# open-mmlab/Live2Diff

Measured on AMD Instinct MI355X. Metric: frames/sec @512×512, 2 denoise steps; per-step latency; 1/2/4/8 GPU, higher is better.
Workload: dtype f16; 1 GPU; BASELINE configs[1]: 512x512 image (64x64 latent), 2 denoise steps, KV window L=16 (8 sink + 8 rolling), SD-1.5 UNet widths + Live2Diff temporal attention, one independent stream per GPU; plan_launches=433, hipgraph=False, device=AMD Radeon Graphics (gfx950:sramecc+:xnack-, 256 CUs), output_finite=True, default_workload=True

## Files before the change

### live2diff_amd/csrc/igemm.hip

```cpp
#include "common.h"

typedef unsigned int u32x4 __attribute__((ext_vector_type(4)));
#define L2D_GPTR(p) ((__attribute__((address_space(1))) const void *)(p))
#define L2D_LPTR(p) ((__attribute__((address_space(3))) void *)(p))

struct IGemmArgs {
    const h16 *w;
    const h16 *zero;
    long long sw;
    int Nout, Kp, nwg, ntn, ntm, order, splitk;
    float inv_ntn, inv_ntm, inv_s;
    const h16 *x1, *x2;
    long long sx1;
    int M, C1, C2, ldx1, ldx2, CinP, B, Hin, Win, Hout, Wout, stride, ups, taps;
    int pad;
    float inv_hw, inv_wout;
    const float *bias, *rowbias;
    const h16 *res;
    h16 *out;
    long long so, sres;
    int ldo, ldr, ldrb, rows_per_bias, epi, epl;
    float *ws;
    unsigned int *cnt;
    unsigned long long *gn1, *gn2;
    int gnT, gnG, cpg1, choff1, cpg2, choff2;
#ifdef L2D_PROBES
    unsigned long long *probe;
#endif
};

#ifdef L2D_PROBES
static unsigned long long *g_igemm_probe = nullptr;
extern "C" void l2d_igemm_set_probe(void *p) { g_igemm_probe = (unsigned long long *)p; }
#define L2D_STAMP(i)                                                                                              \
    do {                                                                                                          \
        if (a.probe && threadIdx.x == 0)                                                                          \
            a.probe[((blockIdx.z * gridDim.y + blockIdx.y) * (unsigned long long)gridDim.x + blockIdx.x) * 8 + (i)] = __builtin_readcyclecounter(); \
    } while (0)
#else
#define L2D_STAMP(i) do { } while (0)
#endif

__device__ __forceinline__ int l2d_divf(int n, int d, float inv) {
    int q = (int)((float)n * inv);
    const int r = n - q * d;
    q += (r >= d ? 1 : 0) - (r < 0 ? 1 : 0);
    return q;
}

__device__ __forceinline__ void igemm_epilogue(const IGemmArgs &a, h16 *outp, const h16 *resp, int m, int n, f32x4 v) {
    const float *rb = a.rowbias ? a.rowbias + (long long)(m / a.rows_per_bias) * a.ldrb : nullptr;
    if (n + 4 > a.Nout) {
#pragma unroll
        for (int r = 0; r < 4; ++r) {
            if (n + r >= a.Nout) break;
            float y = v[r];
            if (a.bias) y += a.bias[n + r];
            if (rb) y += rb[n + r];
            if (a.epi == 2) y = l2d_silu(y);
            if (a.epi == 3) y = fmaxf(y, 0.f);
            if (a.epi == 5) y = l2d_gelu(y);
            if (resp) y += (float)resp[(long long)m * a.ldr + n + r];
            if (a.epi == 4) y = fmaxf(y, 0.f);
            outp[(long long)m * a.ldo + n + r] = (h16)y;
        }
        return;
    }
    if (a.bias) v += *reinterpret_cast<const f32x4 *>(a.bias + n);
    if (rb) v += *reinterpret_cast<const f32x4 *>(rb + n);
    if (a.epi == 2) {
#pragma unroll
        for (int r = 0; r < 4; ++r) v[r] = l2d_silu(v[r]);
    }
    if (a.epi == 3) {
#pragma unroll
        for (int r = 0; r < 4; ++r) v[r] = fmaxf(v[r], 0.f);
    }
    if (a.epi == 5) {
#pragma unroll
        for (int r = 0; r < 4; ++r) v[r] = l2d_gelu(v[r]);
    }
    if (resp) {
        h16x4 rr = *reinterpret_cast<const h16x4 *>(resp + (long long)m * a.ldr + n);
#pragma unroll
        for (int r = 0; r < 4; ++r) v[r] += (float)rr[r];
    }
    if (a.epi == 4) {
#pragma unroll
        for (int r = 0; r < 4; ++r) v[r] = fmaxf(v[r], 0.f);
    }
    h16x4 o;
#pragma unroll
    for (int r = 0; r < 4; ++r) o[r] = (h16)v[r];
    *reinterpret_cast<h16x4 *>(outp + (long long)m * a.ldo + n) = o;
}

template <int TN, int TM, int MODE, int BK, int NS>
__global__ __launch_bounds__(256, (TN == 128 && BK == 32) ? (NS == 2 ? 4 : 3) : 1) void igemm_kernel(IGemmArgs a) {
    constexpr int NI = TN / 32;
    constexpr int MI = TM / 32;
    constexpr int SPR = BK / 8;
    constexpr int RPI = 64 / SPR;
    constexpr int NIW = TN / RPI / 4;
    constexpr int NIX = TM / RPI / 4;
    constexpr int LPS = NIW + NIX;
    constexpr int KK = BK / 32;
    constexpr int STAGE = (TN + TM) * BK;
    extern __shared__ __attribute__((aligned(16))) h16 smem[];

    unsigned ka0, ka1, ka2, ka3;
    {
        const auto kp = __builtin_amdgcn_kernarg_segment_ptr();
        static_assert(sizeof(IGemmArgs) > 0xc0 + 4, "argument block shrank: adjust the warm-up offsets");
        asm volatile("s_load_dword %0, %4, 0x0\n\ts_load_dword %1, %4, 0x40\n\ts_load_dword %2, %4, 0x80\n\ts_load_dword %3, %4, 0xc0"
                     : "=&s"(ka0), "=&s"(ka1), "=&s"(ka2), "=&s"(ka3)
                     : "s"(kp));
    }
    L2D_STAMP(0);
    const int tid = threadIdx.x;
    const int lane = tid & 63;
    const int wave = __builtin_amdgcn_readfirstlane(tid >> 6);
    const int wn = wave >> 1, wm = wave & 1;
    const int li = lane & 15, lg = lane >> 4;
    auto swz = [](int r) { return BK == 32 ? ((r >> 1) & 3) : (BK == 64 ? (r & 7) : (r & 15)); };

// ... 180 lines not shown
        if (resp) {
#pragma unroll
            for (int it = 0; it < EPI_IT; ++it) {
                const int c = it * 256 + tid, row = c / CPRN, cc = c % CPRN;
                const int m = m0 + row, n = n0 + cc * 8;
                resv[RES_EARLY ? it : 0] = (m < a.M && n < a.Nout) ? l2d_ld8(resp + (long long)m * a.ldr + n) : l2d_zero8();
            }
        }
    };
    if (vec && RES_EARLY && !split) load_early();
    if (kb < ke) issue_x();

    f32x4 acc[NI][MI];
#pragma unroll
    for (int i = 0; i < NI; ++i)
#pragma unroll
        for (int j = 0; j < MI; ++j) acc[i][j] = (f32x4){0.f, 0.f, 0.f, 0.f};

    int aoff[KK][NI], boff[KK][MI];
#pragma unroll
    for (int kk = 0; kk < KK; ++kk) {
#pragma unroll
        for (int i = 0; i < NI; ++i) {
            const int r = wn * (TN / 2) + i * 16 + li;
            aoff[kk][i] = r * BK + (((kk * 4 + lg) ^ swz(r)) << 3);
        }
#pragma unroll
        for (int j = 0; j < MI; ++j) {
            const int r = wm * (TM / 2) + j * 16 + li;
            boff[kk][j] = (TN + r) * BK + (((kk * 4 + lg) ^ swz(r)) << 3);
        }
    }
    int cp_slot = 0;
    auto compute = [&]() {
        const h16 *st = smem + cp_slot * STAGE;
#pragma unroll
        for (int kk = 0; kk < KK; ++kk) {
            h16x8 af[NI], bf[MI];
#pragma unroll
            for (int i = 0; i < NI; ++i) af[i] = l2d_ld8(st + aoff[kk][i]);
#pragma unroll
            for (int j = 0; j < MI; ++j) bf[j] = l2d_ld8(st + boff[kk][j]);
#pragma unroll
            for (int i = 0; i < NI; ++i)
#pragma unroll
                for (int j = 0; j < MI; ++j)
                    acc[i][j] = __builtin_amdgcn_mfma_f32_16x16x32_f16(af[i], bf[j], acc[i][j], 0, 0, 0);
        }
        cp_slot = (cp_slot + 1 == NS) ? 0 : cp_slot + 1;
    };

#pragma unroll
    for (int s = 1; s < NS - 1; ++s)
        if (kb + s < ke) issue();
    L2D_STAMP(2);
    int kt = kb;
    for (; kt + (NS - 1) < ke; ++kt) {
        asm volatile("s_waitcnt vmcnt(%0)" ::"n"((NS - 2) * LPS) : "memory");
        __builtin_amdgcn_s_barrier();
        if (kt == kb) L2D_STAMP(3);
        issue();
        compute();
    }
    for (; kt < ke; ++kt) {
        asm volatile("s_waitcnt vmcnt(0)" ::: "memory");
        __builtin_amdgcn_s_barrier();
        compute();
    }

    L2D_STAMP(4);
    if (split && a.cnt) {
        const int S = a.splitk;
        constexpr int AUX_SC1 = 16;
        float *slab = a.ws + ((z * nwg + wgid) * S) * (long long)(TN * TM);
        const __amdgpu_buffer_rsrc_t rs = __builtin_amdgcn_make_buffer_rsrc(slab, 0, S * TN * TM * 4, 0x00020000);
        const int mine = ((int)blockIdx.y * (TN * TM) + tid * 4) * 4;
#pragma unroll
        for (int j = 0; j < MI; ++j) {
            if (m0 + wm * (TM / 2) + j * 16 >= a.M) continue;
#pragma unroll
            for (int i = 0; i < NI; ++i)
                __builtin_amdgcn_raw_buffer_store_b128(__builtin_bit_cast(u32x4, acc[i][j]), rs, mine + (i * MI + j) * 4096, 0, AUX_SC1);
        }
        asm volatile("s_waitcnt vmcnt(0)" ::: "memory");
        __syncthreads();
        unsigned int *flag = reinterpret_cast<unsigned int *>(smem);
        if (tid == 0) *flag = atomicAdd(a.cnt + (z * nwg + wgid), 1u);
        __syncthreads();
        const bool last = (*flag == (unsigned int)(S - 1));
        __syncthreads();
        if (!last) return;
        if (tid == 0) atomicExch(a.cnt + (z * nwg + wgid), 0u);
#pragma unroll
        for (int i = 0; i < NI; ++i)
#pragma unroll
            for (int j = 0; j < MI; ++j) acc[i][j] = (f32x4){0.f, 0.f, 0.f, 0.f};
#pragma unroll
        for (int j = 0; j < MI; ++j) {
            if (m0 + wm * (TM / 2) + j * 16 >= a.M) continue;
#pragma unroll 4
            for (int y = 0; y < S; ++y) {
                const int src = (y * (TN * TM) + tid * 4) * 4;
#pragma unroll
                for (int i = 0; i < NI; ++i)
                    acc[i][j] += __builtin_bit_cast(f32x4, __builtin_amdgcn_raw_buffer_load_b128(rs, src + (i * MI + j) * 4096, 0, AUX_SC1));
            }
        }
        if (vec && RES_EARLY) load_early();
    } else if (split) {
        const int NoutP = (a.Nout + 3) & ~3;
        float *wsp = a.ws + ((long long)z * a.splitk + blockIdx.y) * a.M * NoutP;
#pragma unroll
        for (int j = 0; j < MI; ++j) {
            const int m = m0 + wm * (TM / 2) + j * 16 + li;
            if (m >= a.M) continue;
#pragma unroll
            for (int i = 0; i < NI; ++i) {
                const int n = n0 + wn * (TN / 2) + i * 16 + lg * 4;
                if (n >= a.Nout) continue;
                *reinterpret_cast<f32x4 *>(wsp + (long long)m * NoutP + n) = acc[i][j];
            }
        }
        return;
    }
    if (vec) {
        const int pitch = (a.epi == 1 ? TN / 2 : TN) + 8;
        h16 *ot = smem;
        if (!RES_EARLY) load_bias();
        __syncthreads();
        if (a.epi == 1) {
#pragma unroll
            for (int j = 0; j < MI; ++j) {
                const int row = wm * (TM / 2) + j * 16 + li;
#pragma unroll
                for (int p = 0; p < NI / 2; ++p) {
                    const int col = wn * (TN / 4) + p * 16 + lg * 4;
                    h16x4 o;
#pragma unroll
                    for (int r = 0; r < 4; ++r) {
                        const float v = acc[2 * p][j][r] + biasv[2 * p][r];
                        const float g = acc[2 * p + 1][j][r] + biasv[2 * p + 1][r];
                        o[r] = (h16)(v * l2d_gelu(g));
                    }
                    *reinterpret_cast<h16x4 *>(ot + row * pitch + col) = o;
                }
            }
        } else {
#pragma unroll
            for (int j = 0; j < MI; ++j) {
                const int row = wm * (TM / 2) + j * 16 + li;
                const float *rb = (a.rowbias && !rb_in_bias)
                                      ? a.rowbias + (long long)((m0 + row < a.M ? m0 + row : a.M - 1) / a.rows_per_bias) * a.ldrb
                                      : nullptr;
#pragma unroll
                for (int i = 0; i < NI; ++i) {
                    const int col = wn * (TN / 2) + i * 16 + lg * 4;
                    f32x4 v = acc[i][j] + biasv[i];
                    if constexpr (RES_EARLY) v += rbv[i];
                    if (rb && n0 + col < a.Nout) v += *reinterpret_cast<const f32x4 *>(rb + n0 + col);
                    if (a.epi == 2) {
#pragma unroll
                        for (int r = 0; r < 4; ++r) v[r] = l2d_silu(v[r]);
                    }
                    if (a.epi == 3) {
#pragma unroll
                        for (int r = 0; r < 4; ++r) v[r] = fmaxf(v[r], 0.f);
                    }
                    if (a.epi == 5) {
#pragma unroll
                        for (int r = 0; r < 4; ++r) v[r] = l2d_gelu(v[r]);
                    }
                    h16x4 o;
#pragma unroll
                    for (int r = 0; r < 4; ++r) o[r] = (h16)v[r];
                    *reinterpret_cast<h16x4 *>(ot + row * pitch + col) = o;
                }
            }
        }
        constexpr int CPRN_LOG = (CPRN == 16) ? 4 : 3;
        const int cshift = (a.epi == 1) ? CPRN_LOG - 1 : CPRN_LOG;
        const int n0o = (a.epi == 1) ? (n0 >> 1) : n0;
        L2D_STAMP(5);
        h16x8 rlate[RES_EARLY ? 1 : EPI_IT];
        if (!RES_EARLY && resp) {
#pragma unroll
            for (int it = 0; it < EPI_IT; ++it) {
                const int c = it * 256 + tid, row = c / CPRN, cc = c % CPRN;
                const int m = m0 + row, n = n0 + cc * 8;
                rlate[it] = (m < a.M && n < a.Nout) ? l2d_ld8(resp + (long long)m * a.ldr + n) : l2d_zero8();
            }
        }
// ... 255 lines not shown
```

### live2diff_amd/csrc/rowgemm.hip

```cpp
#include <type_traits>

#include "common.h"

typedef float f32x16 __attribute__((ext_vector_type(16)));

struct RowGemmArgs {
    const h16 *x, *w;
    const float *bias;
    const h16 *res;
    h16 *out, *outT;
    const long long *gnacc;
    unsigned long long *gn1, *gn2;
    long long sT;
    int M, K, Nout, ldx, ldo, ldr, ldt;
    int epi, pro, T, G, cpg;
    int nm, ny, ytr, tr_n0, order;
    int gnT, gnG, cpg1, choff1, cpg2, choff2;
    float eps, inv_cpg;
#ifdef L2D_PROBES
    unsigned long long *probe;
#endif
};

#ifdef L2D_PROBES
// ... 188 lines not shown
    for (int e = 0; e < 4; ++e) { gs[e] = 0.f; gq[e] = 0.f; }
    const h16x2 ones2 = {(h16)1.0f, (h16)1.0f};
#pragma unroll
    for (int it = 0; it < EIT; ++it) {
        const int row = rr + it * RPP;
        if (!on || row >= BM || m0 + row >= a.M) continue;
        h16x8 v = l2d_ld8(os + row * pitch + cc * 8);
        if (a.res) {
            if constexpr (RES_PRE) v = v + resv[it];
            else v = v + l2d_ld8(a.res + (long long)(m0 + row) * a.ldr + nb_o + cc * 8);
        }
        l2d_st8_out<L2D_WT_ROWGEMM>(a.out + (long long)(m0 + row) * a.ldo + nb_o + cc * 8, v);
        if (gn) {
#pragma unroll
            for (int e = 0; e < 4; ++e) {
                const h16x2 pr = {v[2 * e], v[2 * e + 1]};
                gs[e] = __builtin_amdgcn_fdot2(pr, ones2, gs[e], false);
                gq[e] = __builtin_amdgcn_fdot2(pr, pr, gq[e], false);
            }
        }
    }
    RG_STAMP(6);
    if (gn) {
        float *red = reinterpret_cast<float *>(smem + BM * pitch);
#pragma unroll
        for (int e = 0; e < 4; ++e) { red[tid * 8 + e] = gs[e]; red[tid * 8 + 4 + e] = gq[e]; }
        __syncthreads();
        float *chs1 = red + nthr * 8, *chs2 = chs1 + (BNo >> 1);
        if (tid < (BNo >> 1)) {
            const int c8 = tid >> 2, e = tid & 3;
            float s = 0.f, q = 0.f;
            for (int r = 0; r < RPP; ++r) { s += red[(r * CPR + c8) * 8 + e]; q += red[(r * CPR + c8) * 8 + 4 + e]; }
            chs1[tid] = s; chs2[tid] = q;
        }
        __syncthreads();
        const int bsmp = m0 / a.gnT;
        l2d_gn_flush(a.gn1, a.gnG, a.cpg1 >> 1, a.choff1 >> 1, bsmp, chs1, chs2, nb_o >> 1, BNo >> 1, tid);
        l2d_gn_flush(a.gn2, a.gnG, a.cpg2 >> 1, a.choff2 >> 1, bsmp, chs1, chs2, nb_o >> 1, BNo >> 1, tid);
    }
}

template <int NT, int MT, int RD, int SK, int MAXT>
__global__ __launch_bounds__(MAXT) void rowgemm_kernel(RowGemmArgs a) {
    constexpr int BM = 32 * MT;
    extern __shared__ __attribute__((aligned(16))) h16 smem[];
    const int tid = threadIdx.x, lane = tid & 63;
    const int nthr = blockDim.x, NW = nthr >> 6;
    const int wave = __builtin_amdgcn_readfirstlane(tid >> 6);
    RG_STAMP(0);

    const int nwg = a.nm * a.ny;
    int wgid;
    {
        const int q = nwg >> 3, r = nwg & 7, xcd = blockIdx.x & 7, idx = blockIdx.x >> 3;
        wgid = (xcd < r ? xcd * (q + 1) : r * (q + 1) + (xcd - r) * q) + idx;
    }
    int mtile, y;
    if (a.order) { y = wgid / a.nm; mtile = wgid - y * a.nm; }
    else { mtile = wgid / a.ny; y = wgid - mtile * a.ny; }
    const int m0 = mtile * BM;
    const int S = SK > 0 ? SK : (a.K >> 4);
    const int KK = SK > 0 ? SK * 16 : a.K;
    const int t0 = (y * NW + wave) * NT;

    const h16 *wp = a.w + (long long)t0 * S * 512;
    const int wlane = lane * 8;
    const long long tstride = (long long)S * 512;
    constexpr int RING = rg_ring<RD, SK>();
    h16x8 wr[RING][NT];
    auto request_ring = [&]() {
        long long ro = 0;
#pragma unroll
        for (int s = 0; s < RING; ++s) {
            asm volatile("" : "+s"(ro));
#pragma unroll
            for (int i = 0; i < NT; ++i) wr[s][i] = l2d_ld8(wp + (ro + i * tstride) + wlane);
            ro += 512;
        }
        __builtin_amdgcn_sched_barrier(0);
    };
    RG_STAMP(1);

    float *tab = reinterpret_cast<float *>(smem + BM * KK + 8 * BM);
    if (a.pro == 2) {
        float *rstd_s = tab + 2 * KK, *shf_s = rstd_s + 32;
        if (tid < a.G) {
            const long long *src = a.gnacc + ((long long)(m0 / a.T) * a.G + tid) * 2;
            const float s = (float)((double)src[0] * (1.0 / 1048576.0));
            const float q = (float)((double)src[1] * (1.0 / 4096.0));
            const float inv = 1.0f / ((float)a.T * (float)a.cpg);
            const float mean = s * inv;
            const float var = fmaxf(q * inv - mean * mean, 0.f);
            const float rstd = rsqrtf(var + a.eps);
            rstd_s[tid] = rstd;
            shf_s[tid] = -mean * rstd;
        }
        __syncthreads();
        for (int c = tid; c < KK; c += nthr) {
            const int g = (int)(((float)c + 0.5f) * a.inv_cpg);
            tab[c] = rstd_s[g];
            tab[KK + c] = shf_s[g];
        }
        __syncthreads();
    }

    RG_STAMP(2);
    {
        constexpr int XG = 10;
        const bool wide = nthr >= 16 * BM && (KK & 127) == 0;
        const int lsh = wide ? 4 : 3, LPR = 1 << lsh;
        const int KS = KK >> (3 + lsh);
        const int nch = (KS + XG - 1) / XG;
        const int j = tid & (LPR - 1);
        const int dstep = 8 * LPR * BM;
        const int r0 = tid >> lsh, rstep = nthr >> lsh;
        const bool has_row = r0 < BM;
        const int r_last = has_row ? r0 + ((BM - 1 - r0) / rstep) * rstep : 0;
        const bool ln_reg = a.pro == 1 && nch == 1;

        auto load_group = [&](h16x8 (&v)[XG], int r, int i0) {
            const int m = m0 + r;
            const h16 *src = a.x + (long long)(m < a.M ? m : 0) * a.ldx + j * 8;
#pragma unroll
            for (int u = 0; u < XG; ++u) v[u] = l2d_ld8(src + (i0 + u < KS ? i0 + u : KS - 1) * (8 * LPR));
            __builtin_amdgcn_sched_barrier(0);
        };
        auto consume_group = [&](h16x8 (&v)[XG], int r, int i0, float &s) {
            const bool rv = m0 + r < a.M;
            h16 *dst = smem + (j * BM + (r ^ (2 * (j & 7)))) * 8;
            if (ln_reg) {
                float t = 0.f;
#pragma unroll
                for (int u = 0; u < XG; ++u) {
                    if (u >= KS) break;
                    if (!rv) v[u] = l2d_zero8();
#pragma unroll
                    for (int e = 0; e < 8; ++e) t += (float)v[u][e];
                }
                const float mean = rg_row_sum(t, wide) / (float)KK;
                float q = 0.f;
#pragma unroll
                for (int u = 0; u < XG; ++u) {
                    if (u >= KS) break;
#pragma unroll
                    for (int e = 0; e < 8; ++e) { const float d = (float)v[u][e] - mean; q += d * d; }
                }
                const float rstd = rsqrtf(rg_row_sum(q, wide) / (float)KK + a.eps);
#pragma unroll
                for (int u = 0; u < XG; ++u) {
                    if (u >= KS) break;
                    h16x8 o;
#pragma unroll
                    for (int e = 0; e < 8; ++e) o[e] = (h16)(((float)v[u][e] - mean) * rstd);
                    l2d_st8(dst + u * dstep, o);
                }
                return;
            }
#pragma unroll
            for (int u = 0; u < XG; ++u) {
                if (i0 + u >= KS) break;
                if (!rv) v[u] = l2d_zero8();
                if (a.pro == 2) {
                    const int c0 = (j + LPR * (i0 + u)) * 8;
                    const f32x4 sa = *reinterpret_cast<const f32x4 *>(tab + c0), sb = *reinterpret_cast<const f32x4 *>(tab + c0 + 4);
                    const f32x4 ha = *reinterpret_cast<const f32x4 *>(tab + KK + c0), hb = *reinterpret_cast<const f32x4 *>(tab + KK + c0 + 4);
                    h16x8 o;
#pragma unroll
                    for (int e = 0; e < 4; ++e) {
                        o[e] = (h16)((float)v[u][e] * sa[e] + ha[e]);
                        o[4 + e] = (h16)((float)v[u][4 + e] * sb[e] + hb[e]);
                    }
                    v[u] = rv ? o : l2d_zero8();
                } else if (a.pro == 1) {
#pragma unroll
                    for (int e = 0; e < 8; ++e) s += (float)v[u][e];
                }
                l2d_st8(dst + (i0 + u) * dstep, v[u]);
            }
        };
        auto finish_row_lds = [&](int r, float s) {
            h16 *dst = smem + (j * BM + (r ^ (2 * (j & 7)))) * 8;
            const float mean = rg_row_sum(s, wide) / (float)KK;
            float q = 0.f;
#pragma unroll 5
            for (int i = 0; i < KS; ++i) {
                const h16x8 v = l2d_ld8(dst + i * dstep);
#pragma unroll
                for (int e = 0; e < 8; ++e) { const float d = (float)v[e] - mean; q += d * d; }
            }
            const float rstd = rsqrtf(rg_row_sum(q, wide) / (float)KK + a.eps);
#pragma unroll 5
            for (int i = 0; i < KS; ++i) {
                const h16x8 v = l2d_ld8(dst + i * dstep);
                h16x8 o;
#pragma unroll
                for (int e = 0; e < 8; ++e) o[e] = (h16)(((float)v[e] - mean) * rstd);
                l2d_st8(dst + i * dstep, o);
            }
        };

        float srow = 0.f;
        if (has_row) {
            for (int r = r0; r < BM; r += rstep) {
                const int ng = (r == r_last) ? nch - 1 : nch;
                for (int c = 0; c < ng; ++c) {
                    h16x8 v[XG];
                    load_group(v, r, c * XG);
                    consume_group(v, r, c * XG, srow);
                }
                if (r != r_last) {
                    if (a.pro == 1 && !ln_reg) finish_row_lds(r, srow);
                    srow = 0.f;
                }
            }
        }
        h16x8 vl[XG];
        if (has_row) load_group(vl, r_last, (nch - 1) * XG);
        request_ring();
        if (has_row) {
            consume_group(vl, r_last, (nch - 1) * XG, srow);
            if (a.pro == 1 && !ln_reg) finish_row_lds(r_last, srow);
        }
    }
    __syncthreads();
    RG_STAMP(3);
    rowgemm_body<NT, MT, RD, SK>(a, smem, wr, wp, wlane, tstride, S, m0, y, NW, wave, lane, tid, nthr);
}

template <int NT, int MT, int RD, int SK, int MAXT>
static void launch_rg(const RowGemmArgs &a, int nthr, size_t lds, hipStream_t s) {
    static bool attr_done_dev[L2D_MAX_DEV] = {false};
    bool &attr_done = attr_done_dev[l2d_dev_ordinal()];
    if (lds > 65536 && !attr_done) {
        if (hipFuncSetAttribute((const void *)rowgemm_kernel<NT, MT, RD, SK, MAXT>, hipFuncAttributeMaxDynamicSharedMemorySize, 163840) == hipSuccess)
            attr_done = true;
        else
            (void)hipGetLastError();
    }
    hipLaunchKernelGGL((rowgemm_kernel<NT, MT, RD, SK, MAXT>), dim3(a.nm * a.ny), dim3(nthr), lds, s, a);
}

template <int NT, int MT, int RD, int MAXT>
static void launch_k(const RowGemmArgs &a, int nthr, size_t lds, hipStream_t s) {
    switch (a.K) {
        case 320: launch_rg<NT, MT, RD, 20, MAXT>(a, nthr, lds, s); break;
        case 640: launch_rg<NT, MT, RD, 40, MAXT>(a, nthr, lds, s); break;
        case 1280: launch_rg<NT, MT, RD, 80, MAXT>(a, nthr, lds, s); break;
        default: launch_rg<NT, MT, RD, 0, MAXT>(a, nthr, lds, s); break;
    }
}

int l2d_launch_rowgemm(const l2d_op *op, hipStream_t s) {
    RowGemmArgs a;
    a.x = (const h16 *)op->p[0]; a.w = (const h16 *)op->p[1]; a.bias = (const float *)op->p[2]; a.res = (const h16 *)op->p[3];
    a.out = (h16 *)op->p[4]; a.gnacc = (const long long *)op->p[7];
    a.outT = (h16 *)op->p[8];
    a.gn1 = (unsigned long long *)op->p[9]; a.gn2 = (unsigned long long *)op->p[10];
    a.M = op->i[0]; a.K = op->i[1]; a.Nout = op->i[2]; a.ldx = op->i[3]; a.ldo = op->i[4]; a.ldr = op->i[5];
    a.epi = op->i[6]; a.pro = op->i[7]; a.T = op->i[9]; a.G = op->i[10];
    const int NW = op->i[12], NT = op->i[13], MT = op->i[14];
    const int ntr = op->i[15];
    a.ldt = op->i[16]; a.order = op->i[17] ? 1 : 0;
    a.sT = op->l[0];
    a.eps = op->f[0];
#ifdef L2D_PROBES
    a.probe = g_rowgemm_probe;
#endif
    a.gnT = op->i[24]; a.gnG = op->i[25]; a.cpg1 = op->i[26]; a.choff1 = op->i[27]; a.cpg2 = op->i[28]; a.choff2 = op->i[29];
    if (!a.gn1 && a.gn2) { a.gn1 = a.gn2; a.cpg1 = a.cpg2; a.choff1 = a.choff2; a.gn2 = nullptr; }
    const int BM = 32 * MT;
    const int tiles = a.Nout > 0 ? a.Nout / 32 : 0;
    const bool geom_ok = NW >= 1 && NW <= (NT >= 3 ? 5 : 8) && NT >= 1 && NT <= 4 && (MT == 1 || MT == 2 || MT == 4) &&
                         !(MT >= 2 && NT > 2) && !(MT == 4 && a.K != 320) &&
                         tiles > 0 && (a.Nout % 32) == 0 && (tiles % (NW * NT)) == 0 && ntr >= 0 && ntr <= tiles &&
                         (ntr % (NW * NT)) == 0;
    if (!a.x || !a.w || a.M <= 0 || a.K <= 0 || (a.K % 64) || a.K > 2048 || !geom_ok || (a.ldx % 8) || a.ldx < a.K ||
        a.epi < 0 || a.epi > 1 || a.pro < 0 || a.pro > 2 ||
        (ntr < tiles && (!a.out || (a.ldo % 8))) || (a.res && (a.ldr % 8)) ||
        (a.epi == 1 && (!a.bias || a.res || ntr != 0)) ||
        (a.pro == 2 && (!a.gnacc || a.T <= 0 || (a.T % BM) || (a.M % a.T) || a.G <= 0 || a.G > 32 || (a.K % a.G))) ||
        (ntr > 0 && (!a.outT || a.T <= 0 || (a.T % BM) || (a.M % a.T) || (a.ldt % 8) || a.ldt < a.T)) ||
        (((unsigned long long)a.x | (unsigned long long)a.w | (unsigned long long)a.out | (unsigned long long)a.res |
          (unsigned long long)a.outT | (unsigned long long)a.bias) & 15)) {
        l2d_set_error("rowgemm(tag %d): invalid arguments (M=%d K=%d Nout=%d ldx=%d ldo=%d epi=%d pro=%d NW=%d NT=%d MT=%d ntr=%d T=%d)",
                      op->tag, a.M, a.K, a.Nout, a.ldx, a.ldo, a.epi, a.pro, NW, NT, MT, ntr, a.T);
        return L2D_EINVAL;
    }
    const int BNp = NW * NT * 32, BNo = a.epi == 1 ? BNp / 2 : BNp, nthr = 64 * NW;
    if (a.gn1) {
        if (a.gnT <= 0 || (a.gnT % BM) || (a.M % a.gnT) || a.gnG <= 0 || a.gnG > 32 || a.cpg1 <= 0 || (a.gn2 && a.cpg2 <= 0) ||
            ((a.cpg1 | a.choff1) & 1) || (a.gn2 && ((a.cpg2 | a.choff2) & 1)) || ntr != 0 || a.epi == 1 || nthr < 32) {
            l2d_set_error("rowgemm(tag %d): GroupNorm statistics need T %% %d == 0 (T=%d), even group sizes and offsets, no "
                          "transposed part", op->tag, BM, a.gnT);
            return L2D_EINVAL;
        }
    }
    a.cpg = a.pro == 2 ? a.K / a.G : 1;
    a.inv_cpg = 1.0f / (float)a.cpg;
    a.nm = (a.M + BM - 1) / BM;
    a.ny = tiles / (NW * NT);
// ... 28 lines not shown
```

### live2diff_amd/csrc/wsgemm.hip

```cpp
#include <type_traits>

#include "common.h"

typedef float f32x16 __attribute__((ext_vector_type(16)));
typedef unsigned int u32x4 __attribute__((ext_vector_type(4)));

#define L2D_GPTR(p) ((__attribute__((address_space(1))) const void *)(p))
#define L2D_LPTR(p) ((__attribute__((address_space(3))) void *)(p))

struct WsArgs {
    const h16 *x1, *x2, *w, *zero;
    const float *bias, *colsum, *rowbias;
    const h16 *res;
    h16 *out, *outT;
    float *ws;
    unsigned int *cnt;
    unsigned long long *gn1, *gn2;
    long long sT;
    int M, Ktot, C1, C2, CinP, ldx1, ldx2, ldo, ldr, ldt, ldrb, rows_per_bias;
    int taps, H, W, T;
    float invT, invW;
    int epi, pro;
    int nm, ny, S, cps, crem, ncpt, ytr, tr_n0;
    int gnT, gnG, cpg1, choff1, cpg2, choff2;
// ... 296 lines not shown
                if constexpr (REFILL) {
                    const int kn = ks + 4 * RDS;
                    const int kk = kn < ks_last ? kn : ks_last;
#pragma unroll
                    for (int i = 0; i < NT; ++i) ws_gload<NTW>(wr[j][i], voff[i], wp + (long long)kk * 512);
                }
                ++ks;
                __builtin_amdgcn_sched_barrier(0);
            };
            auto step = [&](auto uc) {
                constexpr int u = decltype(uc)::value;
                const unsigned ad = xoff[u + 1] + sbr;
                ws_lread<sb>(xf[(u + 1) & 1][0], ad); ws_lread<sb + 4096>(xf[(u + 1) & 1][1], ad);
                ws_lread<sb + 8192>(xf[(u + 1) & 1][2], ad); ws_lread<sb + 12288>(xf[(u + 1) & 1][3], ad);
                ws_lwait<4>(xf[u & 1][0], xf[u & 1][1], xf[u & 1][2], xf[u & 1][3]);
                __builtin_amdgcn_sched_barrier(0);
                compute(uc);
            };
            step(std::integral_constant<int, 0>{});
            step(std::integral_constant<int, 1>{});
            step(std::integral_constant<int, 2>{});
            ws_lwait<0>(xf[1][0], xf[1][1], xf[1][2], xf[1][3]);
            __builtin_amdgcn_s_barrier();
            {
                const unsigned ad = xoff[0] + nbr;
                ws_lread<nb>(xf[0][0], ad); ws_lread<nb + 4096>(xf[0][1], ad); ws_lread<nb + 8192>(xf[0][2], ad); ws_lread<nb + 12288>(xf[0][3], ad);
            }
            __builtin_amdgcn_sched_barrier(0);
            compute(std::integral_constant<int, 3>{});
            ws_lwait<0>(xf[0][0], xf[0][1], xf[0][2], xf[0][3]);
#ifdef L2D_PROBES
            { const int sdone = (ks >> 2) - c0 - 1; if (wave == 0 && sdone < 12) WS_STAMP(35 + 2 * sdone); }
#endif
        };
        using T_ = std::true_type;
        using F_ = std::false_type;
#define WS_C(v) std::integral_constant<int, (v)>{}
        auto tail = [&](auto base_c, int s0, int rem) {
            constexpr int B0 = decltype(base_c)::value;
#define WS_SL(k) WS_C(B0 < 0 ? -1 : ((B0 + (k)) & (NS - 1))), ((s0 + (k)) & (NS - 1))
            do_stage(WS_C(0), F_{}, WS_SL(0));
            if constexpr (RDS > 1) {
                if (rem > 1) {
                    do_stage(WS_C(1), F_{}, WS_SL(1));
                    if constexpr (RDS > 2) {
                        if (rem > 2) {
                            do_stage(WS_C(2), F_{}, WS_SL(2));
                            if constexpr (RDS > 3) {
                                if (rem > 3) do_stage(WS_C(3), F_{}, WS_SL(3));
                            }
                        }
                    }
                }
            }
#undef WS_SL
        };
        static_assert(RDS == NS || 2 * RDS == NS, "the k loop is written for a register ring of NS or NS / 2 stages");
        int s = 0;
        if constexpr (RDS == NS) {
            for (; s + RDS < n; s += RDS) {
                do_stage(WS_C(0), T_{}, WS_C(0), 0);
                do_stage(WS_C(1), T_{}, WS_C(1), 0);
                do_stage(WS_C(2), T_{}, WS_C(2), 0);
                do_stage(WS_C(3), T_{}, WS_C(3), 0);
            }
            tail(WS_C(0), 0, n - s);
        } else {
            for (; s + RDS < n; s += RDS) {
                do_stage(WS_C(0), T_{}, WS_C(-1), s & (NS - 1));
                do_stage(WS_C(1), T_{}, WS_C(-1), (s + 1) & (NS - 1));
            }
            tail(WS_C(-1), s, n - s);
        }
#pragma unroll
        for (int i = 0; i < NT; ++i)
#pragma unroll
            for (int j = 0; j < 4 * RDS; j += 8)
                ws_gdrain8(wr[j][i], wr[j + 1][i], wr[j + 2][i], wr[j + 3][i], wr[j + 4][i], wr[j + 5][i], wr[j + 6][i], wr[j + 7][i]);
#undef WS_C
        if (wave == 0) WS_STAMP(60);
    }

    if constexpr (!RES_EARLY) request_residual();
    __syncthreads();
    if (wave == 0) WS_STAMP(61);

    if (a.S > 1) {
        constexpr int AUX_SC1 = 16;
        const int SLABF = BM * BNp + 2 * BM;
        const int tile = y * a.nm + mtile;
        float *slab = a.ws + (long long)tile * a.S * SLABF;
        const __amdgpu_buffer_rsrc_t rs = __builtin_amdgcn_make_buffer_rsrc(slab, 0, a.S * SLABF * 4, 0x00020000);
        if (cons) {
#pragma unroll
            for (int i = 0; i < NT; ++i)
#pragma unroll
                for (int mt = 0; mt < MT; ++mt)
#pragma unroll
                    for (int e4 = 0; e4 < 4; ++e4) {
                        const f32x4 v = {acc[i][mt][4 * e4], acc[i][mt][4 * e4 + 1], acc[i][mt][4 * e4 + 2], acc[i][mt][4 * e4 + 3]};
                        __builtin_amdgcn_raw_buffer_store_b128(__builtin_bit_cast(u32x4, v), rs,
                                                               (z * SLABF + ((((wave * NT + i) * MT + mt) * 4 + e4) * 256)) * 4 + lane * 16, 0, AUX_SC1);
                    }
            if (a.pro == 1 && tid < 64) {
                const f32x4 v = *reinterpret_cast<const f32x4 *>(stat + tid * 4);
                __builtin_amdgcn_raw_buffer_store_b128(__builtin_bit_cast(u32x4, v), rs, (z * SLABF + BM * BNp) * 4 + tid * 16, 0, AUX_SC1);
            }
        }
        asm volatile("s_waitcnt vmcnt(0)" ::: "memory");
        __syncthreads();
        unsigned int *flag = reinterpret_cast<unsigned int *>(stat + 2 * BM);
        if (tid == 0) *flag = atomicAdd(a.cnt + tile, 1u);
        __syncthreads();
        const bool last = (*flag == (unsigned int)(a.S - 1));
        if (wave == 0) WS_STAMP(62);
        if (!last) return;
        if (tid == 0) atomicExch(a.cnt + tile, 0u);
        if (cons) {
#pragma unroll
            for (int i = 0; i < NT; ++i)
#pragma unroll
                for (int mt = 0; mt < MT; ++mt)
#pragma unroll
                    for (int e = 0; e < 16; ++e) acc[i][mt][e] = 0.f;
            for (int zz = 0; zz < a.S; ++zz) {
#pragma unroll
                for (int i = 0; i < NT; ++i)
#pragma unroll
                    for (int mt = 0; mt < MT; ++mt)
#pragma unroll
                        for (int e4 = 0; e4 < 4; ++e4) {
                            const f32x4 v = __builtin_bit_cast(f32x4, __builtin_amdgcn_raw_buffer_load_b128(
                                rs, (zz * SLABF + ((((wave * NT + i) * MT + mt) * 4 + e4) * 256)) * 4 + lane * 16, 0, AUX_SC1));
#pragma unroll
                            for (int e = 0; e < 4; ++e) acc[i][mt][4 * e4 + e] += v[e];
                        }
            }
            if (a.pro == 1 && tid < 64) {
                f32x4 t = {0.f, 0.f, 0.f, 0.f};
                for (int zz = 0; zz < a.S; ++zz)
                    t += __builtin_bit_cast(f32x4, __builtin_amdgcn_raw_buffer_load_b128(rs, (zz * SLABF + BM * BNp) * 4 + tid * 16, 0, AUX_SC1));
                *reinterpret_cast<f32x4 *>(stat + tid * 4) = t;
            }
        }
        __syncthreads();
    }

    if (a.pro == 1) {
        if (tid < BM) {
            const float inv = 1.0f / (float)a.Ktot;
            const float mean = stat[2 * tid] * inv;
            const float var = fmaxf(stat[2 * tid + 1] * inv - mean * mean, 0.f);
            const float rstd = rsqrtf(var + a.eps);
            stat[2 * tid] = rstd;
            stat[2 * tid + 1] = -mean * rstd;
        }
        __syncthreads();
    }

    h16 *os = smem;
    if (y >= a.ytr) {
        const int pt = BM + 8;
        if (cons) {
#pragma unroll
            for (int i = 0; i < NT; ++i) {
                const int tp = (wave * NT + i) * 32;
#pragma unroll
                for (int g4 = 0; g4 < 4; ++g4) {
                    const int ch = tp + 8 * g4 + 4 * lh;
                    f32x4 bb = {0.f, 0.f, 0.f, 0.f}, cs = {0.f, 0.f, 0.f, 0.f};
                    if (a.bias) bb = *reinterpret_cast<const f32x4 *>(par + ch);
                    if (a.pro == 1) cs = *reinterpret_cast<const f32x4 *>(par + WS_PSTR + ch);
#pragma unroll
                    for (int mt = 0; mt < MT; ++mt) {
                        float rsd = 1.f, nmr = 0.f;
                        if (a.pro == 1) { rsd = stat[(32 * mt + l32) * 2]; nmr = stat[(32 * mt + l32) * 2 + 1]; }
#pragma unroll
                        for (int e = 0; e < 4; ++e)
                            os[(tp + 8 * g4 + 4 * lh + e) * pt + 32 * mt + l32] = (h16)(acc[i][mt][4 * g4 + e] * rsd + nmr * cs[e] + bb[e]);
                    }
                }
            }
        }
        __syncthreads();
        if (cons) {
            const int b = m0 / a.T, tb = m0 - b * a.T;
            h16 *ob = a.outT + (long long)b * a.sT + (long long)(nb_p - a.tr_n0) * a.ldt + tb;
            constexpr int CPT = BM / 8;
            for (int idx = tid; idx < BNp * CPT; idx += nthr) {
                const int ch = idx / CPT, c = idx - ch * CPT;
                l2d_st8_out<L2D_WT_WSGEMM>(ob + (long long)ch * a.ldt + c * 8, l2d_ld8(os + ch * pt + c * 8));
            }
        }
        return;
    }

    if (wave == 0) WS_STAMP(59);
    const int pitch = BNo + 8;
    if (cons) {
        float rsd[MT], nmr[MT];
#pragma unroll
// ... 219 lines not shown
```

Before: 134.0 frames/s.

## Streamline split-K reduction: keep own partial in registers, drop barriers, prefetch GN rows

```diff
diff --git a/live2diff_amd/csrc/igemm.hip b/live2diff_amd/csrc/igemm.hip
--- a/live2diff_amd/csrc/igemm.hip
+++ b/live2diff_amd/csrc/igemm.hip
@@ -41,6 +41,8 @@
 #define L2D_STAMP(i) do { } while (0)
 #endif
 
+template <int V> struct l2d_ic { static constexpr int value = V; };
+
 __device__ __forceinline__ int l2d_divf(int n, int d, float inv) {
     int q = (int)((float)n * inv);
     const int r = n - q * d;
@@ -387,31 +389,95 @@
             for (int i = 0; i < NI; ++i)
                 __builtin_amdgcn_raw_buffer_store_b128(__builtin_bit_cast(u32x4, acc[i][j]), rs, mine + (i * MI + j) * 4096, 0, AUX_SC1);
         }
+        if (vec && RES_EARLY) load_early();
         asm volatile("s_waitcnt vmcnt(0)" ::: "memory");
         __syncthreads();
+        L2D_STAMP(1);
         unsigned int *flag = reinterpret_cast<unsigned int *>(smem);
         if (tid == 0) *flag = atomicAdd(a.cnt + (z * nwg + wgid), 1u);
         __syncthreads();
         const bool last = (*flag == (unsigned int)(S - 1));
-        __syncthreads();
+        L2D_STAMP(2);
         if (!last) return;
         if (tid == 0) atomicExch(a.cnt + (z * nwg + wgid), 0u);
-#pragma unroll
-        for (int i = 0; i < NI; ++i)
-#pragma unroll
-            for (int j = 0; j < MI; ++j) acc[i][j] = (f32x4){0.f, 0.f, 0.f, 0.f};
-#pragma unroll
-        for (int j = 0; j < MI; ++j) {
-            if (m0 + wm * (TM / 2) + j * 16 >= a.M) continue;
+        const int zy = (int)blockIdx.y, NF = S - 1;
+        constexpr bool SMALLT = (TN * TM <= 64 * 64);
+        constexpr int JB = MI, FB = 4;
+        if constexpr (!SMALLT) {
+#pragma unroll
+            for (int i = 0; i < NI; ++i)
+#pragma unroll
+                for (int j = 0; j < MI; ++j) acc[i][j] = (f32x4){0.f, 0.f, 0.f, 0.f};
+#pragma unroll
+            for (int j = 0; j < MI; ++j) {
+                if (m0 + wm * (TM / 2) + j * 16 >= a.M) continue;
 #pragma unroll 4
-            for (int y = 0; y < S; ++y) {
-                const int src = (y * (TN * TM) + tid * 4) * 4;
-#pragma unroll
-                for (int i = 0; i < NI; ++i)
-                    acc[i][j] += __builtin_bit_cast(f32x4, __builtin_amdgcn_raw_buffer_load_b128(rs, src + (i * MI + j) * 4096, 0, AUX_SC1));
-            }
-        }
-        if (vec && RES_EARLY) load_early();
+                for (int y = 0; y < S; ++y) {
+                    const int src = (y * (TN * TM) + tid * 4) * 4;
+#pragma unroll
+                    for (int i = 0; i < NI; ++i)
+                        acc[i][j] += __builtin_bit_cast(f32x4, __builtin_amdgcn_raw_buffer_load_b128(rs, src + (i * MI + j) * 4096, 0, AUX_SC1));
+                }
+            }
+        } else {
+#pragma unroll
+        for (int j0 = 0; j0 < MI; j0 += JB) {
+            f32x4 t[JB][NI];
+#pragma unroll
+            for (int jj = 0; jj < JB; ++jj)
+#pragma unroll
+                for (int i = 0; i < NI; ++i) t[jj][i] = (f32x4){0.f, 0.f, 0.f, 0.f};
+            auto trip = [&](auto nb, int f0) {
+                constexpr int NB = decltype(nb)::value;
+                u32x4 fr[NB][JB][NI];
+#pragma unroll
+                for (int b = 0; b < NB; ++b) {
+                    const int y = f0 + b + (f0 + b >= zy ? 1 : 0);
+                    const int src = (y * (TN * TM) + tid * 4) * 4;
+#pragma unroll
+                    for (int jj = 0; jj < JB; ++jj) {
+                        if (m0 + wm * (TM / 2) + (j0 + jj) * 16 >= a.M) continue;
+#pragma unroll
+                        for (int i = 0; i < NI; ++i)
+                            fr[b][jj][i] = __builtin_amdgcn_raw_buffer_load_b128(rs, src + (i * MI + j0 + jj) * 4096, 0, AUX_SC1);
+                    }
+                }
+                __builtin_amdgcn_sched_barrier(0);
+#pragma unroll
+                for (int b = 0; b < NB; ++b) {
+                    const bool own_here = (f0 + b == zy);
+#pragma unroll
+                    for (int jj = 0; jj < JB; ++jj) {
+                        if (m0 + wm * (TM / 2) + (j0 + jj) * 16 >= a.M) continue;
+#pragma unroll
+                        for (int i = 0; i < NI; ++i) {
+                            const f32x4 to = t[jj][i] + acc[i][j0 + jj];
+                            t[jj][i] = own_here ? to : t[jj][i];
+                            t[jj][i] += __builtin_bit_cast(f32x4, fr[b][jj][i]);
+                        }
+                    }
+                }
+            };
+            int f = 0;
+            for (; f + FB <= NF; f += FB) trip(l2d_ic<FB>{}, f);
+            switch (NF - f) {
+            case 1: trip(l2d_ic<1>{}, f); break;
+            case 2: trip(l2d_ic<2>{}, f); break;
+            case 3: trip(l2d_ic<3>{}, f); break;
+            default: break;
+            }
+#pragma unroll
+            for (int jj = 0; jj < JB; ++jj) {
+                const bool beyond = m0 + wm * (TM / 2) + (j0 + jj) * 16 >= a.M;
+#pragma unroll
+                for (int i = 0; i < NI; ++i) {
+                    const f32x4 to = t[jj][i] + acc[i][j0 + jj];
+                    acc[i][j0 + jj] = beyond ? (f32x4){0.f, 0.f, 0.f, 0.f} : (zy == NF ? to : t[jj][i]);
+                }
+            }
+        }
+        }
+        L2D_STAMP(3);
     } else if (split) {
         const int NoutP = (a.Nout + 3) & ~3;
         float *wsp = a.ws + ((long long)z * a.splitk + blockIdx.y) * a.M * NoutP;
diff --git a/live2diff_amd/csrc/rowgemm.hip b/live2diff_amd/csrc/rowgemm.hip
--- a/live2diff_amd/csrc/rowgemm.hip
+++ b/live2diff_amd/csrc/rowgemm.hip
@@ -294,7 +294,7 @@
     RG_STAMP(1);
 
     float *tab = reinterpret_cast<float *>(smem + BM * KK + 8 * BM);
-    if (a.pro == 2) {
+    auto gn_tables = [&]() {
         float *rstd_s = tab + 2 * KK, *shf_s = rstd_s + 32;
         if (tid < a.G) {
             const long long *src = a.gnacc + ((long long)(m0 / a.T) * a.G + tid) * 2;
@@ -314,9 +314,8 @@
             tab[KK + c] = shf_s[g];
         }
         __syncthreads();
-    }
-
-    RG_STAMP(2);
+    };
+
     {
         constexpr int XG = 10;
         const bool wide = nthr >= 16 * BM && (KK & 127) == 0;
@@ -411,13 +410,24 @@
             }
         };
 
+        const bool early = a.pro == 2 && rstep >= BM;
+        h16x8 ve[XG];
+        if (early && has_row) load_group(ve, r0, 0);
+        if (a.pro == 2) gn_tables();
+        RG_STAMP(2);
+
         float srow = 0.f;
         if (has_row) {
             for (int r = r0; r < BM; r += rstep) {
                 const int ng = (r == r_last) ? nch - 1 : nch;
                 for (int c = 0; c < ng; ++c) {
                     h16x8 v[XG];
-                    load_group(v, r, c * XG);
+                    if (early && c == 0) {
+#pragma unroll
+                        for (int u = 0; u < XG; ++u) v[u] = ve[u];
+                    } else {
+                        load_group(v, r, c * XG);
+                    }
                     consume_group(v, r, c * XG, srow);
                 }
                 if (r != r_last) {
@@ -427,7 +437,14 @@
             }
         }
         h16x8 vl[XG];
-        if (has_row) load_group(vl, r_last, (nch - 1) * XG);
+        if (has_row) {
+            if (early && nch == 1) {
+#pragma unroll
+                for (int u = 0; u < XG; ++u) vl[u] = ve[u];
+            } else {
+                load_group(vl, r_last, (nch - 1) * XG);
+            }
+        }
         request_ring();
         if (has_row) {
             consume_group(vl, r_last, (nch - 1) * XG, srow);
diff --git a/live2diff_amd/csrc/wsgemm.hip b/live2diff_amd/csrc/wsgemm.hip
--- a/live2diff_amd/csrc/wsgemm.hip
+++ b/live2diff_amd/csrc/wsgemm.hip
@@ -402,7 +402,7 @@
     }
 
     if constexpr (!RES_EARLY) request_residual();
-    __syncthreads();
+    if (a.S == 1 || a.pro == 1) __syncthreads();
     if (wave == 0) WS_STAMP(61);
 
     if (a.S > 1) {
@@ -429,6 +429,7 @@
         }
         asm volatile("s_waitcnt vmcnt(0)" ::: "memory");
         __syncthreads();
+        if (wave == 0) WS_STAMP(56);
         unsigned int *flag = reinterpret_cast<unsigned int *>(stat + 2 * BM);
         if (tid == 0) *flag = atomicAdd(a.cnt + tile, 1u);
         __syncthreads();
@@ -436,7 +437,50 @@
         if (wave == 0) WS_STAMP(62);
         if (!last) return;
         if (tid == 0) atomicExch(a.cnt + tile, 0u);
-        if (cons) {
+        auto sum_slabs = [&](auto sc) {
+            constexpr int SC = decltype(sc)::value;
+            constexpr int OOB = 0x40000000;
+            int vb[SC];
+#pragma unroll
+            for (int zz = 0; zz < SC; ++zz) vb[zz] = (zz == z) ? OOB : zz * SLABF * 4;
+            if (cons) {
+#pragma unroll
+                for (int i = 0; i < NT; ++i)
+#pragma unroll
+                    for (int mt = 0; mt < MT; ++mt)
+#pragma unroll
+                        for (int e4 = 0; e4 < 4; ++e4) {
+                            const f32x4 mine = {acc[i][mt][4 * e4], acc[i][mt][4 * e4 + 1], acc[i][mt][4 * e4 + 2], acc[i][mt][4 * e4 + 3]};
+                            f32x4 t = {0.f, 0.f, 0.f, 0.f};
+#pragma unroll
+                            for (int zz = 0; zz < SC; ++zz) {
+                                const f32x4 v = __builtin_bit_cast(f32x4, __builtin_amdgcn_raw_buffer_load_b128(
+                                    rs, vb[zz] + ((((wave * NT + i) * MT + mt) * 4 + e4) * 256) * 4 + lane * 16, 0, AUX_SC1));
+                                t += (zz == z) ? mine : v;
+                            }
+#pragma unroll
+                            for (int e = 0; e < 4; ++e) acc[i][mt][4 * e4 + e] = t[e];
+                        }
+                if (a.pro == 1 && tid < 64) {
+                    const f32x4 mine = *reinterpret_cast<const f32x4 *>(stat + tid * 4);
+                    f32x4 t = {0.f, 0.f, 0.f, 0.f};
+#pragma unroll
+                    for (int zz = 0; zz < SC; ++zz) {
+                        const f32x4 v = __builtin_bit_cast(f32x4, __builtin_amdgcn_raw_buffer_load_b128(rs, vb[zz] + BM * BNp * 4 + tid * 16, 0, AUX_SC1));
+                        t += (zz == z) ? mine : v;
+                    }
+                    *reinterpret_cast<f32x4 *>(stat + tid * 4) = t;
+                }
+            }
+        };
+        bool summed = false;
+        if constexpr (NT == 1 && MAXW <= 6) {
+            summed = a.S <= 4;
+            if (a.S == 2) sum_slabs(std::integral_constant<int, 2>{});
+            else if (a.S == 3) sum_slabs(std::integral_constant<int, 3>{});
+            else if (a.S == 4) sum_slabs(std::integral_constant<int, 4>{});
+        }
+        if (!summed && cons) {
 #pragma unroll
             for (int i = 0; i < NT; ++i)
 #pragma unroll
```

Result: no change. 134.1 frames/s, median of 3 (+0.1%).
